# GitHubOfAndrew/TeAMOFlow

Hardware: AMD Instinct MI355X
Metric: train_interactions_per_sec (higher is better)
Workload: dtype f32

## Files before the change

### teamoflow_amd/csrc/tmf_wmrb.hip

```cpp
#include <math.h>
#include <stdlib.h>

#include <type_traits>

#include "tmf_common.h"

namespace tmf {

constexpr int kThreads = 256;
constexpr int kWaves = kThreads / 64;
constexpr int kPosChunk = 512;
constexpr int kUnrollW = 4;
constexpr int kG4Unroll = 4;

__host__ __device__ inline int round4(int x) { return (x + 3) & ~3; }

__host__ __device__ inline int sp_padded(int S) {
    const int nf4 = (S + 3) / 4;
    const int per = ((nf4 + 2 * kWaves - 1) / (2 * kWaves) + 1) & ~1;
    return 4 * 2 * kWaves * per;
}

__device__ __forceinline__ void count_ge0_x4(int& c0, int& c1, float x0, float x1, float x2, float x3) {
    unsigned long long m0, m1, m2, m3;
// ... 973 lines not shown
                       D, delta, (const T*)U_old, U_out, epi, adam, b, e, sy, lag)
        TMF_DISPATCH(T, geom, CALL);
#undef CALL
    }
    return check_launch("tmf_wmrb_gradu4");
}


namespace tmf {
constexpr int kS5Users = 256;
constexpr int kS5Waves = 15;
constexpr int kS5Pad = INT32_MIN;
constexpr int kS5MaxWindows = 4096;
constexpr int kS5Stride = 16;

struct S5Pace {
    const int32_t* wst;
    int* cnt;
    int nw, lag;
};

template <int NV, typename T>
__global__ __launch_bounds__(64 * (kS5Waves + 1)) void k_wmrb_scores5(const int32_t* __restrict__ ids, const int32_t* __restrict__ outs,
                                                                     const int64_t* __restrict__ wg_ptr, int64_t wg0, int64_t n_users,
                                                                     const T* __restrict__ U, const T* __restrict__ V,
                                                                     float* __restrict__ sp, float* __restrict__ p, S5Pace pace) {
    constexpr int G = 32, NGB = 2 * kS5Waves;
    constexpr uint32_t RB = RowBytes<G, NV, T>::value;
    extern __shared__ __attribute__((aligned(16))) char smem_raw[];
    __shared__ int s_win[kS5Waves];
    __shared__ int s_gate;
    int* wst = reinterpret_cast<int*>(smem_raw + (size_t)kS5Users * RB);
    const int tid = threadIdx.x, lane = tid & 63, wave = tid >> 6, g = lane & (G - 1), gid = tid / G;
    const int64_t wg = wg0 + blockIdx.x;
    const int64_t ubeg = wg * kS5Users;
    const int nu = (int)((n_users - ubeg < kS5Users) ? n_users - ubeg : kS5Users);
    const bool paced = pace.cnt != nullptr;
    {
        const tmf_f4* src = reinterpret_cast<const tmf_f4*>(reinterpret_cast<const char*>(U) + ubeg * (int64_t)RB);
        tmf_f4* dst = reinterpret_cast<tmf_f4*>(smem_raw);
        for (int i = tid; i < nu * (int)(RB / 16); i += 64 * (kS5Waves + 1)) dst[i] = __builtin_nontemporal_load(src + i);
        if (paced)
            for (int i = tid; i <= pace.nw; i += 64 * (kS5Waves + 1)) wst[i] = pace.wst[wg * (pace.nw + 1) + i];
        if (tid < kS5Waves) s_win[tid] = 0;
        if (tid == 0) s_gate = paced ? pace.lag : INT32_MAX;
    }
    __syncthreads();
    if (wave == kS5Waves) {
        if (!paced) return;
        const int x = blockIdx.x & 7, peers = ((int)gridDim.x - x + 7) / 8;
        int* cnt = pace.cnt + (size_t)x * pace.nw * kS5Stride;
        int published = 0, gate = pace.lag, idle = 0;
        bool open = false;
        for (;;) {
            int mn = (lane < kS5Waves) ? __hip_atomic_load(&s_win[lane], __ATOMIC_RELAXED, __HIP_MEMORY_SCOPE_WORKGROUP) : INT32_MAX;
#pragma unroll
            for (int o = 8; o >= 1; o >>= 1) mn = min(mn, __shfl_xor(mn, o, 64));
            mn = __builtin_amdgcn_readfirstlane(mn);
            const bool done = mn == INT32_MAX;
            const int target = done ? pace.nw : mn;
            if (lane == 0)
                for (int w = published; w < target; ++w) __hip_atomic_fetch_add(cnt + (size_t)w * kS5Stride, 1, __ATOMIC_RELAXED, __HIP_MEMORY_SCOPE_AGENT);
            if (target > published) published = target;
            if (done) return;
            if (!open && gate < pace.nw - 1) {
                int c = (lane == 0) ? __hip_atomic_load(cnt + (size_t)(gate - pace.lag) * kS5Stride, __ATOMIC_RELAXED, __HIP_MEMORY_SCOPE_AGENT) : 0;
                c = __builtin_amdgcn_readfirstlane(c);
                if (c >= peers) {
                    ++gate;
                    idle = 0;
                    if (lane == 0) __hip_atomic_store(&s_gate, gate, __ATOMIC_RELAXED, __HIP_MEMORY_SCOPE_WORKGROUP);
                    continue;
                }
                if (++idle > 4000) {
                    open = true;
                    if (lane == 0) __hip_atomic_store(&s_gate, INT32_MAX, __ATOMIC_RELAXED, __HIP_MEMORY_SCOPE_WORKGROUP);
                }
            }
            __builtin_amdgcn_s_sleep(4);
        }
    }
    const int64_t beg = wg_ptr[wg], end = wg_ptr[wg + 1];
    const int steps = (int)((end - beg) >> 3);
    const uint32_t loff = 16u * (uint32_t)g;
    const int my_entry = Reduce8x32::entry_of_lane(lane);
    const bool owner = Reduce8x32::owner(lane);
    const int4* id4 = reinterpret_cast<const int4*>(ids + beg);
    const int32_t* out8 = outs + beg + my_entry;
    const int mine = steps > gid ? (steps - gid + NGB - 1) / NGB : 0;
    const int rounds = __builtin_amdgcn_readfirstlane(mine);
    if (rounds > 0) {
        const int last = mine > 0 ? gid + NGB * (mine - 1) : 0;
        struct Ids {
            int4 a, b;
            int o;
        };
        auto fetch = [&](int i) {
            const int st = gid + NGB * i;
            const int sc = st <= last ? st : last;
            Ids r{id4[2 * sc], id4[2 * sc + 1], out8[8 * sc]};
            if (i >= mine) r.o = kS5Pad;
            return r;
        };
        int cur_w = 0, next_b = paced ? wst[1] : INT32_MAX;
        auto pace_to = [&](int i) {
            if (!paced || i >= rounds || cur_w >= pace.nw - 1) return;
            const int st_w = __builtin_amdgcn_readfirstlane(gid + NGB * i);
            if (st_w < next_b) return;
            do {
                ++cur_w;
                next_b = wst[cur_w + 1];
            } while (st_w >= next_b && cur_w < pace.nw - 1);
            if (lane == 0) __hip_atomic_store(&s_win[wave], cur_w, __ATOMIC_RELAXED, __HIP_MEMORY_SCOPE_WORKGROUP);
            for (int spin = 0; spin < 20000; ++spin) {
                if (__hip_atomic_load(&s_gate, __ATOMIC_RELAXED, __HIP_MEMORY_SCOPE_WORKGROUP) >= cur_w) break;
                __builtin_amdgcn_s_sleep(2);
            }
        };
        auto gather = [&](Raw<NV, T> (&y)[8], const Ids& d) {
            const int idv[8] = {d.a.x, d.a.y, d.a.z, d.a.w, d.b.x, d.b.y, d.b.z, d.b.w};
#pragma unroll
            for (int t = 0; t < 8; ++t) load_raw32<G, NV>(y[t], V, (uint32_t)idv[t] & 0xffffffu, loff);
        };
        auto finish = [&](const Raw<NV, T> (&y)[8], const Ids& d) {
            const int idv[8] = {d.a.x, d.a.y, d.a.z, d.a.w, d.b.x, d.b.y, d.b.z, d.b.w};
            float pr[8];
#pragma unroll
            for (int t = 0; t < 8; ++t) {
                Raw<NV, T> x;
                const char* xr = smem_raw + ((uint32_t)idv[t] >> 24) * RB + loff;
                if constexpr (std::is_same<T, float>::value) {
#pragma unroll
                    for (int v = 0; v < NV; ++v) x.v[v] = *reinterpret_cast<const float4*>(xr + 16 * G * v);
                } else {
#pragma unroll
                    for (int pv = 0; pv < NV / 2; ++pv) x.v[pv] = *reinterpret_cast<const bf16x8*>(xr + 16 * G * pv);
                }
                pr[t] = dot_raw<NV>(x, y[t]);
            }
            const float sc = Reduce8x32::run(pr, lane);
            if (owner && d.o != kS5Pad) __builtin_nontemporal_store(sc, d.o >= 0 ? sp + d.o : p + ~d.o);
        };
        Raw<NV, T> yA[8], yB[8];
        Ids A = fetch(0);
        Ids B = fetch(1);
        pace_to(0);
        gather(yA, A);
        for (int i = 0; i < rounds; i += 2) {
            Ids C = fetch(i + 2);
            __builtin_amdgcn_sched_barrier(0);
            pace_to(i + 1);
            gather(yB, B);
            __builtin_amdgcn_sched_barrier(0);
            finish(yA, A);
            __builtin_amdgcn_sched_barrier(0);
            if (i + 1 >= rounds) break;
            Ids Dn = fetch(i + 3);
            __builtin_amdgcn_sched_barrier(0);
            pace_to(i + 2);
            gather(yA, C);
            __builtin_amdgcn_sched_barrier(0);
            finish(yB, B);
            __builtin_amdgcn_sched_barrier(0);
            A = C;
            B = Dn;
        }
    }
    if (lane == 0) __hip_atomic_store(&s_win[wave], INT32_MAX, __ATOMIC_RELAXED, __HIP_MEMORY_SCOPE_WORKGROUP);
}

}

namespace tmf {
constexpr int kS6Users = 64;
constexpr int kS6Waves = 8;

template <int NV, typename T>
__global__ __launch_bounds__(64 * kS6Waves) void k_wmrb_scores6(const int32_t* __restrict__ ids, const int32_t* __restrict__ outs,
                                                                const int64_t* __restrict__ chunk_ptr, int64_t chunk0, int64_t n_groups,
                                                                int64_t n_users, const T* __restrict__ U, const T* __restrict__ V,
                                                                float* __restrict__ sp, float* __restrict__ p) {
    constexpr int G = 32, NGB = 2 * kS6Waves;
    constexpr uint32_t RB = RowBytes<G, NV, T>::value;
    __shared__ __attribute__((aligned(16))) char smem_raw[kS6Users * RB];
    const int tid = threadIdx.x, lane = tid & 63, g = lane & (G - 1), gid = tid / G;
    const int64_t chunk = chunk0 + blockIdx.x;
    const int64_t beg = chunk_ptr[chunk], end = chunk_ptr[chunk + 1];
    if (beg == end) return;
    const int64_t ubeg = (chunk % n_groups) * kS6Users;
    const int nu = (int)((n_users - ubeg < kS6Users) ? n_users - ubeg : kS6Users);
    {
        const tmf_f4* src = reinterpret_cast<const tmf_f4*>(reinterpret_cast<const char*>(U) + ubeg * (int64_t)RB);
        tmf_f4* dst = reinterpret_cast<tmf_f4*>(smem_raw);
        for (int i = tid; i < nu * (int)(RB / 16); i += 64 * kS6Waves) dst[i] = __builtin_nontemporal_load(src + i);
    }
    __syncthreads();
    const int steps = (int)((end - beg) >> 3);
    const uint32_t loff = 16u * (uint32_t)g;
    const int my_entry = Reduce8x32::entry_of_lane(lane);
    const bool owner = Reduce8x32::owner(lane);
    const int4* id4 = reinterpret_cast<const int4*>(ids + beg);
    const int32_t* out8 = outs + beg + my_entry;
    const int mine = steps > gid ? (steps - gid + NGB - 1) / NGB : 0;
    const int rounds = __builtin_amdgcn_readfirstlane(mine);
    if (rounds == 0) return;
    const int last = mine > 0 ? gid + NGB * (mine - 1) : 0;
    struct Ids {
        int4 a, b;
        int o;
    };
    auto fetch = [&](int i) {
        const int st = gid + NGB * i;
        const int sc = st <= last ? st : last;
        Ids r{id4[2 * sc], id4[2 * sc + 1], out8[8 * sc]};
        if (i >= mine) r.o = kS5Pad;
        return r;
    };
    auto gather = [&](Raw<NV, T> (&y)[8], const Ids& d) {
        const int idv[8] = {d.a.x, d.a.y, d.a.z, d.a.w, d.b.x, d.b.y, d.b.z, d.b.w};
#pragma unroll
        for (int t = 0; t < 8; ++t) load_raw32<G, NV>(y[t], V, (uint32_t)idv[t] & 0xffffffu, loff);
    };
    auto finish = [&](const Raw<NV, T> (&y)[8], const Ids& d) {
        const int idv[8] = {d.a.x, d.a.y, d.a.z, d.a.w, d.b.x, d.b.y, d.b.z, d.b.w};
        float pr[8];
#pragma unroll
        for (int t = 0; t < 8; ++t) {
            Raw<NV, T> x;
            const char* xr = smem_raw + ((uint32_t)idv[t] >> 24) * RB + loff;
            if constexpr (std::is_same<T, float>::value) {
#pragma unroll
                for (int v = 0; v < NV; ++v) x.v[v] = *reinterpret_cast<const float4*>(xr + 16 * G * v);
            } else {
#pragma unroll
                for (int pv = 0; pv < NV / 2; ++pv) x.v[pv] = *reinterpret_cast<const bf16x8*>(xr + 16 * G * pv);
            }
            pr[t] = dot_raw<NV>(x, y[t]);
        }
        const float sc = Reduce8x32::run(pr, lane);
        if (owner && d.o != kS5Pad) __builtin_nontemporal_store(sc, d.o >= 0 ? sp + d.o : p + ~d.o);
    };
    Raw<NV, T> yA[8];
    Ids A = fetch(0);
    for (int i = 0; i < rounds; ++i) {
        Ids B = fetch(i + 1);
        __builtin_amdgcn_sched_barrier(0);
        gather(yA, A);
        __builtin_amdgcn_sched_barrier(0);
        finish(yA, A);
        A = B;
    }
}

}

static bool s6_supported(int n_components, int bf16, int64_t n_items) {
    const tmf::RowGeom geom = bf16 ? tmf::row_geom_bf16(n_components) : tmf::row_geom(n_components);
    const int64_t row_bytes = (int64_t)geom.ld * (bf16 ? 2 : 4);
    return geom.G == 32 && n_items > 0 && n_items < (1 << 24) && n_items * row_bytes < ((int64_t)1 << 32);
}

template <typename T>
static int wmrb_scores6_impl(const int32_t* ids, const int32_t* outs, const int64_t* chunk_ptr, int64_t n_groups, int32_t n_slices,
                             int64_t n_users, int64_t n_items, const void* U, const void* V, float* sp, float* p, int n_components,
                             void* stream) {
    if (n_users == 0 || n_slices == 0) return TMF_OK;
    const RowGeom geom = row_geom_of<T>(n_components);
    TMF_REQUIRE(ids && outs && chunk_ptr && U && V && sp && p, "wmrb_scores6: null pointer");
    TMF_REQUIRE(n_groups == (n_users + kS6Users - 1) / kS6Users && n_slices > 0, "wmrb_scores6: %lld groups for %lld users (%d per group), %d slices",
                (long long)n_groups, (long long)n_users, kS6Users, n_slices);
    if (!s6_supported(n_components, std::is_same<T, __bf16>::value, n_items)) {
        set_error("wmrb_scores6: needs rows of 32 lanes (fp32 65..128 / bf16 129..256 components) and fewer than 2^24 items in a table "
                  "below 4 GB (got %d components, %lld items)", n_components, (long long)n_items);
        return TMF_E_UNSUPPORTED;
    }
    const int64_t per_slice = n_groups * 64 * kS6Waves;
    const int max_slices = (int)((((int64_t)1 << 32) - 1) / per_slice);
    TMF_REQUIRE(max_slices >= 1, "wmrb_scores6: %lld user groups exceed one launch", (long long)n_groups);
    for (int s0 = 0; s0 < n_slices; s0 += max_slices) {
        const int nsl = (n_slices - s0 < max_slices) ? n_slices - s0 : max_slices;
        const unsigned blocks = (unsigned)(n_groups * nsl);
#define CALL(G_, NV_)                                                                                                       \
    {                                                                                                                       \
        if constexpr (G_ == 32) {                                                                                           \
            hipLaunchKernelGGL((k_wmrb_scores6<NV_, T>), dim3(blocks), dim3(64 * kS6Waves), 0, (hipStream_t)stream, ids, outs, \
                               chunk_ptr, (int64_t)s0 * n_groups, n_groups, n_users, (const T*)U, (const T*)V, sp, p);      \
        }                                                                                                                   \
    }
        TMF_DISPATCH(T, geom, CALL);
#undef CALL
    }
    return check_launch("tmf_wmrb_scores6");
}

namespace tmf {
constexpr int kS7Users = 256;
constexpr int kS7Slots = 6144;
constexpr int kS7K = 4;
constexpr int kS7Waves = 16;
constexpr int kS7Flight = 2;
constexpr uint32_t kS7RowBytes = 512;
constexpr size_t kS7Lds = (size_t)kS7Users * kS7RowBytes + (size_t)(kS7Slots + 64) * sizeof(float);

struct S7Streams {
    const int4* steps;
    const int32_t* place;
    const int64_t* sub_step;
    const int64_t* sub_place;
    const int32_t* chunk_sub;
    const int32_t* sub_wave;
    const int32_t* sub_fill;
};

__global__ __launch_bounds__(64 * kS7Waves) void k_wmrb_scores7(S7Streams a, int64_t chunk0, int64_t n_groups, int64_t n_users,
                                                                const float* __restrict__ U, const float* __restrict__ V,
                                                                float* __restrict__ sp, float* __restrict__ p) {
    constexpr int NG = 8 * kS7Waves, NT = 64 * kS7Waves, FL = kS7Flight;
    extern __shared__ __attribute__((aligned(16))) char smem_raw[];
    float* sbuf = reinterpret_cast<float*>(smem_raw + (size_t)kS7Users * kS7RowBytes);
    const int tid = threadIdx.x, lane = tid & 63, g = lane & 7, gid = tid >> 3;
    const int64_t chunk = chunk0 + blockIdx.x;
    const int sub_b = a.chunk_sub[chunk], sub_e = a.chunk_sub[chunk + 1];
    if (sub_b == sub_e) return;
    const int64_t ubeg = (chunk % n_groups) * kS7Users;
    const int nu = (int)((n_users - ubeg < kS7Users) ? n_users - ubeg : kS7Users);
    {
        const tmf_f4* src = reinterpret_cast<const tmf_f4*>(reinterpret_cast<const char*>(U) + ubeg * (int64_t)kS7RowBytes);
        tmf_f4* dst = reinterpret_cast<tmf_f4*>(smem_raw);
        for (int i = tid; i < nu * (int)(kS7RowBytes / 16); i += NT) dst[i] = __builtin_nontemporal_load(src + i);
    }
    __syncthreads();
    const uint32_t par = (lane >> 4) & 1;
    const uint32_t offA = 16u * g + 128u * par, offB = 16u * g + 128u * (par ^ 1u);
    const uint32_t slot_sel = 0x0c0c0000u | ((2u * (g & 3) + 1u) << 8) | (2u * (g & 3));
    struct Row {
        float4 v[4];
    };
    auto dot = [](const Row& x, const Row& y) {
        float q[4];
#pragma unroll
        for (int v = 0; v < 4; ++v) {
            tmf_f2 a = tmf_f2{x.v[v].x, x.v[v].y} * tmf_f2{y.v[v].x, y.v[v].y};
            a = __builtin_elementwise_fma(tmf_f2{x.v[v].z, x.v[v].w}, tmf_f2{y.v[v].z, y.v[v].w}, a);
            q[v] = a.x + a.y;
        }
        return (q[0] + q[2]) + (q[1] + q[3]);
    };
    auto run = [&](auto fill_tag, const int4* rec0, int first, int stride, int end, int rounds) {
        constexpr int FILL = decltype(fill_tag)::value;
        auto fetch = [&](int i) {
            const int st = first + stride * i;
            return rec0[st < end ? st : end - 1];
        };
        auto gather = [&](Row& y, const int4& r) {
            const char* base = reinterpret_cast<const char*>(V);
            const uint32_t oa = row_byte_off<kS7RowBytes>((uint32_t)r.x, offA), ob = row_byte_off<kS7RowBytes>((uint32_t)r.x, offB);
            y.v[0] = *reinterpret_cast<const float4*>(base + oa);
            y.v[1] = *reinterpret_cast<const float4*>(base + ob);
            y.v[2] = *reinterpret_cast<const float4*>(base + oa + 256);
            y.v[3] = *reinterpret_cast<const float4*>(base + ob + 256);
        };
        auto finish = [&](const Row& y, const int4& r, int i) {
            float s[FILL];
#pragma unroll
            for (int k = 0; k < FILL; ++k) {
                const uint32_t lu = ((uint32_t)r.y >> (8 * k)) & 0xffu;
                const char* xa = smem_raw + (lu * kS7RowBytes + offA);
                const char* xb = smem_raw + (lu * kS7RowBytes + offB);
                Row x;
                x.v[0] = *reinterpret_cast<const float4*>(xa);
                x.v[1] = *reinterpret_cast<const float4*>(xb);
                x.v[2] = *reinterpret_cast<const float4*>(xa + 256);
                x.v[3] = *reinterpret_cast<const float4*>(xb + 256);
                float t = dot(x, y);
                t += TMF_DPP_MOV(t, 0xB1);
                t += TMF_DPP_MOV(t, 0x4E);
                t += TMF_DPP_MOV(t, 0x141);
                s[k] = t;
            }
            float mine_s = s[0];
            if constexpr (FILL == 2) mine_s = (g & 1) ? s[1] : s[0];
            if constexpr (FILL == 3) mine_s = (g & 2) ? s[2] : ((g & 1) ? s[1] : s[0]);
            if constexpr (FILL == 4) mine_s = (g & 2) ? ((g & 1) ? s[3] : s[2]) : ((g & 1) ? s[1] : s[0]);
            uint32_t slot = __builtin_amdgcn_perm((uint32_t)r.w, (uint32_t)r.z, slot_sel);
            slot = (slot < (uint32_t)kS7Slots && first + stride * i < end) ? slot : (uint32_t)kS7Slots;
            if (g < FILL) sbuf[slot] = mine_s;
        };
        Row y[FL];
        int4 rec[2 * FL];
#pragma unroll
        for (int j = 0; j < FL; ++j) rec[j] = fetch(j);
#pragma unroll
        for (int j = 0; j < FL; ++j) {
            gather(y[j], rec[j]);
            rec[FL + j] = fetch(FL + j);
        }
        int i = 0;
        for (; i + 2 * FL <= rounds; i += 2 * FL) {
#pragma unroll
            for (int j = 0; j < 2 * FL; ++j) {
                __builtin_amdgcn_sched_barrier(0);
                finish(y[j % FL], rec[j], i + j);
                __builtin_amdgcn_sched_barrier(0);
                gather(y[j % FL], rec[(j + FL) % (2 * FL)]);
                rec[j] = fetch(i + j + 2 * FL);
            }
        }
        const int rem = rounds - i;
#pragma unroll
        for (int j = 0; j < 2 * FL - 1; ++j) {
            if (j < rem) {
                __builtin_amdgcn_sched_barrier(0);
                finish(y[j % FL], rec[j], i + j);
                __builtin_amdgcn_sched_barrier(0);
                if (j + FL < rem) gather(y[j % FL], rec[j + FL]);
            }
        }
    };
    const int wave = __builtin_amdgcn_readfirstlane(tid >> 6);
    const bool by_fill = a.sub_wave != nullptr;
    for (int sub = sub_b; sub < sub_e; ++sub) {
        const int64_t st0 = a.sub_step[sub];
        const int nsteps = (int)(a.sub_step[sub + 1] - st0);
        const int64_t pl0 = a.sub_place[sub];
        const int nslots = (int)(a.sub_place[sub + 1] - pl0);
        const int4* rec0 = a.steps + st0;
        const int32_t* pl = a.place + pl0;
        int32_t where[kS7Slots / NT];
#pragma unroll
        for (int q = 0; q < kS7Slots / NT; ++q) where[q] = (tid + NT * q < nslots) ? __builtin_nontemporal_load(pl + tid + NT * q) : 0;
        int lo = 8 * wave, hi = nsteps, stride = NG, wb = 0, we = 0, cls = 0;
        if (by_fill) {
            const int32_t* sw = a.sub_wave + (int64_t)sub * (kS7Waves + 1) + wave;
            wb = __builtin_amdgcn_readfirstlane(sw[0]);
            we = __builtin_amdgcn_readfirstlane(sw[1]);
            cls = __builtin_amdgcn_readfirstlane(a.sub_fill[(int64_t)sub * kS7K]);
            lo = wb, hi = we < cls ? we : cls, stride = 8;
        }
        if (lo < hi) run(std::integral_constant<int, 4>{}, rec0, lo + (by_fill ? (gid & 7) : gid - 8 * wave), stride, hi, (hi - lo + stride - 1) / stride);
        if (by_fill) {
            const int32_t* sf = a.sub_fill + (int64_t)sub * kS7K;
            int end = cls + __builtin_amdgcn_readfirstlane(sf[1]);
            lo = wb > cls ? wb : cls, hi = we < end ? we : end, cls = end;
            if (lo < hi) run(std::integral_constant<int, 3>{}, rec0, lo + (gid & 7), 8, hi, (hi - lo + 7) / 8);
            end = cls + __builtin_amdgcn_readfirstlane(sf[2]);
            lo = wb > cls ? wb : cls, hi = we < end ? we : end, cls = end;
            if (lo < hi) run(std::integral_constant<int, 2>{}, rec0, lo + (gid & 7), 8, hi, (hi - lo + 7) / 8);
            lo = wb > cls ? wb : cls, hi = we;
            if (lo < hi) run(std::integral_constant<int, 1>{}, rec0, lo + (gid & 7), 8, hi, (hi - lo + 7) / 8);
        }
        __syncthreads();
#pragma unroll
        for (int q = 0; q < kS7Slots / NT; ++q)
            if (tid + NT * q < nslots)
                __builtin_nontemporal_store(sbuf[tid + NT * q], where[q] >= 0 ? sp + where[q] : p + ~where[q]);
        __syncthreads();
    }
}

}

static bool s7_supported(int n_components, int bf16, int64_t n_items) {
    return !bf16 && n_components >= 65 && n_components <= 128 && s6_supported(n_components, 0, n_items);
}

static int wmrb_scores7_impl(const void* steps, const int32_t* place, const int64_t* sub_step, const int64_t* sub_place,
                             const int32_t* chunk_sub, const int32_t* sub_wave, const int32_t* sub_fill, int64_t n_groups, int32_t n_slices, int64_t n_users, int64_t n_items,
                             const void* U, const void* V, float* sp, float* p, int n_components, void* stream) {
    if (n_users == 0 || n_slices == 0) return TMF_OK;
    TMF_REQUIRE(steps && place && sub_step && sub_place && chunk_sub && U && V && sp && p, "wmrb_scores7: null pointer");
    TMF_REQUIRE(!sub_wave == !sub_fill, "wmrb_scores7: sub_wave and sub_fill come together");
    TMF_REQUIRE(n_groups == (n_users + kS7Users - 1) / kS7Users && n_slices > 0, "wmrb_scores7: %lld groups for %lld users (%d per group), %d slices",
                (long long)n_groups, (long long)n_users, kS7Users, n_slices);
    if (!s7_supported(n_components, 0, n_items)) {
        set_error("wmrb_scores7: needs fp32 rows of 65..128 components and fewer than 2^24 items in a table below 4 GB "
                  "(got %d components, %lld items)", n_components, (long long)n_items);
        return TMF_E_UNSUPPORTED;
    }
    static LdsGrant grant;
    if (int rc = grant_dynamic_lds(reinterpret_cast<const void*>(&k_wmrb_scores7), kS7Lds, grant)) return rc;
    const S7Streams a{static_cast<const int4*>(steps), place, sub_step, sub_place, chunk_sub, sub_wave, sub_fill};
    const int64_t per_slice = n_groups * 64 * kS7Waves;
    const int max_slices = (int)((((int64_t)1 << 32) - 1) / per_slice);
    TMF_REQUIRE(max_slices >= 1, "wmrb_scores7: %lld user groups exceed one launch", (long long)n_groups);
    for (int s0 = 0; s0 < n_slices; s0 += max_slices) {
        const int nsl = (n_slices - s0 < max_slices) ? n_slices - s0 : max_slices;
        hipLaunchKernelGGL(k_wmrb_scores7, dim3((unsigned)(n_groups * nsl)), dim3(64 * kS7Waves), kS7Lds, (hipStream_t)stream, a,
                           (int64_t)s0 * n_groups, n_groups, n_users, (const float*)U, (const float*)V, sp, p);
    }
    return check_launch("tmf_wmrb_scores7");
}

static int s5_launches(int64_t n_wg, int wgs_per_launch) { return (int)((n_wg + wgs_per_launch - 1) / wgs_per_launch); }
static int s5_wgs_per_launch(int wgs_per_launch) {
    if (wgs_per_launch > 0) return wgs_per_launch;
    int dev = 0, cus = 256;
    if (hipGetDevice(&dev) == hipSuccess) (void)hipDeviceGetAttribute(&cus, hipDeviceAttributeMultiprocessorCount, dev);
    return cus > 0 ? cus : 256;
}

template <typename T>
static int wmrb_scores5_impl(const int32_t* ids, const int32_t* outs, const int64_t* wg_ptr, int64_t n_wg, int64_t n_users,
                             int64_t n_items, const void* U, const void* V, float* sp, float* p, int n_components,
                             int wgs_per_launch, const int32_t* wstart, int32_t n_windows, int lag, void* workspace,
                             size_t workspace_bytes, void* stream) {
    if (n_wg == 0 || n_users == 0) return TMF_OK;
    const RowGeom geom = row_geom_of<T>(n_components);
    TMF_REQUIRE(ids && outs && wg_ptr && U && V && sp && p, "wmrb_scores5: null pointer");
    TMF_REQUIRE(n_wg == (n_users + kS5Users - 1) / kS5Users, "wmrb_scores5: %lld workgroups for %lld users (%d per workgroup)",
                (long long)n_wg, (long long)n_users, kS5Users);
    const size_t row_bytes = (size_t)geom.ld * sizeof(T);
    if (geom.G != 32 || row_bytes * kS5Users > 128 * 1024 || n_items <= 0 || n_items >= (1 << 24) ||
        (int64_t)n_items * (int64_t)row_bytes >= ((int64_t)1 << 32)) {
        set_error("wmrb_scores5: needs rows of 32 lanes (fp32 65..128 / bf16 129..256 components) and fewer than 2^24 items "
                  "in a table below 4 GB (got %d components, %lld items)", n_components, (long long)n_items);
        return TMF_E_UNSUPPORTED;
    }
    wgs_per_launch = s5_wgs_per_launch(wgs_per_launch);
    const int launches = s5_launches(n_wg, wgs_per_launch);
    const bool paced = wstart != nullptr && workspace != nullptr && n_windows > 1;
    const size_t per_launch = (size_t)8 * (paced ? n_windows : 0) * kS5Stride * sizeof(int);
    if (paced) {
        TMF_REQUIRE(n_windows <= kS5MaxWindows && lag >= 0, "wmrb_scores5: %d windows (at most %d), lag %d", n_windows, kS5MaxWindows, lag);
        TMF_REQUIRE(workspace_bytes >= per_launch * launches, "wmrb_scores5: workspace of %zu bytes needed, got %zu", per_launch * launches,
                    workspace_bytes);
        if (hipMemsetAsync(workspace, 0, per_launch * launches, (hipStream_t)stream) != hipSuccess) {
            set_error("wmrb_scores5: hipMemsetAsync failed");
            return TMF_E_LAUNCH;
        }
    }
    const size_t lds = row_bytes * kS5Users + (paced ? (size_t)(n_windows + 1) * sizeof(int) : 0);
#define CALL(G_, NV_)                                                                                                       \
    {                                                                                                                       \
        if constexpr (G_ == 32) {                                                                                           \
            static LdsGrant grant;                                                                                          \
            if (int rc = grant_dynamic_lds(reinterpret_cast<const void*>(&k_wmrb_scores5<NV_, T>), lds, grant)) return rc;  \
            for (int l = 0; l < launches; ++l) {                                                                            \
                const int64_t w0 = (int64_t)l * wgs_per_launch;                                                             \
                const unsigned blocks = (unsigned)((n_wg - w0 < wgs_per_launch) ? n_wg - w0 : wgs_per_launch);              \
                const S5Pace pace{wstart, paced ? reinterpret_cast<int*>(static_cast<char*>(workspace) + per_launch * l) : nullptr, \
                                  n_windows, lag};                                                                          \
                hipLaunchKernelGGL((k_wmrb_scores5<NV_, T>), dim3(blocks), dim3(64 * (kS5Waves + 1)), lds, (hipStream_t)stream, \
                                   ids, outs, wg_ptr, w0, n_users, (const T*)U, (const T*)V, sp, p, pace);                  \
            }                                                                                                               \
        }                                                                                                                   \
    }
    TMF_DISPATCH(T, geom, CALL);
#undef CALL
    return check_launch("tmf_wmrb_scores5");
}

template <typename T>
static int wmrb_finish_impl(const float* part, int32_t n_slices, int32_t n_users, const void* U_old, void* U_out,
                            int n_components, int epi, tmf_adam adam, void* stream) {
    if (n_users == 0) return TMF_OK;
    TMF_REQUIRE(part && U_out && n_slices > 0 && (epi == TMF_EPI_GRAD || U_old), "wmrb_finish: bad arguments");
    TMF_REQUIRE(epi == TMF_EPI_ADAM || epi == TMF_EPI_GRAD, "wmrb_finish: bad epilogue %d", epi);
    const RowGeom geom = row_geom_of<T>(n_components);
#define CALL(G_, NV_)                                                                                                  \
    {                                                                                                                  \
        constexpr int per_block = (64 / G_) * kWaves;                                                                  \
        hipLaunchKernelGGL((k_wmrb_finish<G_, NV_, T>), dim3((unsigned)(((int64_t)n_users + per_block - 1) / per_block)), \
                           dim3(kThreads), 0, (hipStream_t)stream, part, (int)n_slices, (int64_t)n_users,                \
                           (const T*)U_old, U_out, epi, adam);                                                         \
    }
    TMF_DISPATCH(T, geom, CALL);
#undef CALL
    return check_launch("tmf_wmrb_finish");
}

#define TMF_SLICED_ENTRY_POINTS(SFX, T_)                                                                                  \
    extern "C" int tmf_wmrb_scores3_##SFX(const tmf_slice_lists* lists, const void* U, const void* V, float* sp, float* p, \
                                          int n_components, void* stream) {                                               \
        return wmrb_scores3_impl<T_>(lists, U, V, sp, p, n_components, stream);                                           \
    }                                                                                                                     \
    extern "C" int tmf_wmrb_scores5_##SFX(const int32_t* ids, const int32_t* outs, const int64_t* wg_ptr, int64_t n_wg,    \
                                          int64_t n_users, int64_t n_items, const void* U, const void* V, float* sp,      \
                                          float* p, int n_components, int wgs_per_launch, const int32_t* wstart,          \
                                          int32_t n_windows, int lag, void* workspace, size_t workspace_bytes,            \
                                          void* stream) {                                                                 \
        return wmrb_scores5_impl<T_>(ids, outs, wg_ptr, n_wg, n_users, n_items, U, V, sp, p, n_components, wgs_per_launch, \
                                     wstart, n_windows, lag, workspace, workspace_bytes, stream);                         \
    }                                                                                                                     \
    extern "C" int tmf_wmrb_scores6_##SFX(const int32_t* ids, const int32_t* outs, const int64_t* chunk_ptr, int64_t n_groups, \
                                          int32_t n_slices, int64_t n_users, int64_t n_items, const void* U, const void* V, \
                                          float* sp, float* p, int n_components, void* stream) {                          \
        return wmrb_scores6_impl<T_>(ids, outs, chunk_ptr, n_groups, n_slices, n_users, n_items, U, V, sp, p, n_components, stream); \
    }                                                                                                                     \
    extern "C" int tmf_wmrb_gradu3_##SFX(const tmf_slice_lists* lists, const float* D, const float* delta,                \
                                         const void* V, float* part, int per_slice_launches, int n_components,            \
                                         void* stream) {                                                                  \
        return wmrb_gradu3_impl<T_>(lists, D, delta, V, part, per_slice_launches, n_components, stream);                  \
    }                                                                                                                     \
    extern "C" int tmf_wmrb_gradu4_##SFX(const tmf_slice_lists* lists, const float* D, const float* delta, const void* V,  \
                                         const void* U_old, void* U_out, int n_components, int epi, tmf_adam adam,       \
                                         int32_t users_per_launch, void* workspace, size_t workspace_bytes, void* stream) { \
        return wmrb_gradu4_impl<T_>(lists, D, delta, V, U_old, U_out, n_components, epi, adam, users_per_launch, workspace, \
                                    workspace_bytes, stream);                                                            \
    }                                                                                                                     \
    extern "C" int tmf_wmrb_finish_##SFX(const float* part, int32_t n_slices, int32_t n_users, const void* U_old,         \
                                         void* U_out, int n_components, int epi, tmf_adam adam, void* stream) {           \
        return wmrb_finish_impl<T_>(part, n_slices, n_users, U_old, U_out, n_components, epi, adam, stream);               \
    }

TMF_SLICED_ENTRY_POINTS(f32, float)
TMF_SLICED_ENTRY_POINTS(bf16, __bf16)

extern "C" int tmf_wmrb_scores6_users_per_group(void) { return tmf::kS6Users; }
extern "C" int tmf_wmrb_scores6_supported(int n_components, int bf16, int64_t n_items) { return s6_supported(n_components, bf16, n_items); }
extern "C" int tmf_wmrb_scores7_f32(const void* steps, const int32_t* place, const int64_t* sub_step, const int64_t* sub_place,
                                    const int32_t* chunk_sub, int64_t n_groups, int32_t n_slices, int64_t n_users, int64_t n_items,
                                    const void* U, const void* V, float* sp, float* p, int n_components, void* stream) {
    return wmrb_scores7_impl(steps, place, sub_step, sub_place, chunk_sub, nullptr, nullptr, n_groups, n_slices, n_users, n_items, U, V, sp, p,
                             n_components, stream);
}
extern "C" int tmf_wmrb_scores7_fill_f32(const void* steps, const int32_t* place, const int64_t* sub_step, const int64_t* sub_place,
                                         const int32_t* chunk_sub, const int32_t* sub_wave, const int32_t* sub_fill, int64_t n_groups,
                                         int32_t n_slices, int64_t n_users, int64_t n_items, const void* U, const void* V, float* sp,
                                         float* p, int n_components, void* stream) {
    TMF_REQUIRE(sub_wave && sub_fill, "wmrb_scores7_fill: null pointer");
    return wmrb_scores7_impl(steps, place, sub_step, sub_place, chunk_sub, sub_wave, sub_fill, n_groups, n_slices, n_users, n_items, U, V,
                             sp, p, n_components, stream);
}
extern "C" int tmf_wmrb_scores7_waves(void) { return tmf::kS7Waves; }
extern "C" int tmf_wmrb_scores7_users_per_group(void) { return tmf::kS7Users; }
extern "C" int tmf_wmrb_scores7_slots(void) { return tmf::kS7Slots; }
extern "C" int tmf_wmrb_scores7_supported(int n_components, int bf16, int64_t n_items) { return s7_supported(n_components, bf16, n_items); }
extern "C" int tmf_wmrb_scores5_users_per_workgroup(void) { return tmf::kS5Users; }
extern "C" size_t tmf_wmrb_scores5_workspace_bytes(int64_t n_wg, int32_t n_windows, int wgs_per_launch) {
    if (n_wg <= 0 || n_windows <= 1) return 0;
    return (size_t)s5_launches(n_wg, s5_wgs_per_launch(wgs_per_launch)) * 8 * (size_t)n_windows * tmf::kS5Stride * sizeof(int);
}
extern "C" int tmf_wmrb_scores5_supported(int n_components, int bf16, int64_t n_items) {
    const tmf::RowGeom geom = bf16 ? tmf::row_geom_bf16(n_components) : tmf::row_geom(n_components);
    const int64_t row_bytes = (int64_t)geom.ld * (bf16 ? 2 : 4);
    return geom.G == 32 && row_bytes * tmf::kS5Users <= 128 * 1024 && n_items > 0 && n_items < (1 << 24) &&
           n_items * row_bytes < ((int64_t)1 << 32);
}
```

Before: 1.270 billion.

## Pipeline WMRB scores7 across sub-chunks with a unified software-pipelined step stream

Replaces the per-sub-chunk run() loops, each with its own prologue and drain, with a single continuous software pipeline. Record fetches and V-row gathers for the next sub-chunk (and the next fill class) are issued while the current one finishes, and the next sub-chunk's placement indices are prefetched before the flush barrier. Sub-chunk metadata comes in through inline scalar-load asm, and the barriers are lighter waitcnt+s_barrier pairs. The aim is to remove pipeline bubbles at sub-chunk and fill-class boundaries. In exchange it adds runtime fill dispatch per step, more register state, and fragile inline asm.

Result: no change. 1.282 billion, median of 6 (+1.0%).

```diff
diff --git a/teamoflow_amd/csrc/tmf_wmrb.hip b/teamoflow_amd/csrc/tmf_wmrb.hip
--- a/teamoflow_amd/csrc/tmf_wmrb.hip
+++ b/teamoflow_amd/csrc/tmf_wmrb.hip
@@ -1299,6 +1299,30 @@
 constexpr uint32_t kS7RowBytes = 512;
 constexpr size_t kS7Lds = (size_t)kS7Users * kS7RowBytes + (size_t)(kS7Slots + 64) * sizeof(float);
 
+__device__ __forceinline__ void s7_open(const int64_t* ss, const int64_t* spl, int64_t& st0, int64_t& st1, int64_t& pl0, int64_t& pl1) {
+    asm volatile("s_load_dwordx2 %0, %4, 0x0\n\ts_load_dwordx2 %1, %4, 0x8\n\ts_load_dwordx2 %2, %5, 0x0\n\ts_load_dwordx2 %3, %5, 0x8\n\t"
+                 "s_waitcnt lgkmcnt(0)"
+                 : "=&s"(st0), "=&s"(st1), "=&s"(pl0), "=&s"(pl1) : "s"(ss), "s"(spl));
+}
+__device__ __forceinline__ void s7_open(const int64_t* ss, const int64_t* spl, const int32_t* sw, const int32_t* sf, int64_t& st0,
+                                        int64_t& pl0, int64_t& pl1, int& wb, int& we, int& n4, int& n3, int& n2) {
+    asm volatile("s_load_dwordx2 %0, %8, 0x0\n\ts_load_dwordx2 %1, %9, 0x0\n\ts_load_dwordx2 %2, %9, 0x8\n\t"
+                 "s_load_dword %3, %10, 0x0\n\ts_load_dword %4, %10, 0x4\n\t"
+                 "s_load_dword %5, %11, 0x0\n\ts_load_dword %6, %11, 0x4\n\ts_load_dword %7, %11, 0x8\n\ts_waitcnt lgkmcnt(0)"
+                 : "=&s"(st0), "=&s"(pl0), "=&s"(pl1), "=&s"(wb), "=&s"(we), "=&s"(n4), "=&s"(n3), "=&s"(n2)
+                 : "s"(ss), "s"(spl), "s"(sw), "s"(sf));
+}
+__device__ __forceinline__ void s7_words(const int64_t* ptr, int64_t& x, int64_t& y) {
+    asm volatile("s_load_dwordx2 %0, %2, 0x0\n\ts_load_dwordx2 %1, %2, 0x8\n\ts_waitcnt lgkmcnt(0)" : "=&s"(x), "=&s"(y) : "s"(ptr));
+}
+
+__device__ __forceinline__ void s7_barrier() {
+    asm volatile("" ::: "memory");
+    __builtin_amdgcn_s_waitcnt(0xc07f);
+    __builtin_amdgcn_s_barrier();
+    asm volatile("" ::: "memory");
+}
+
 struct S7Streams {
     const int4* steps;
     const int32_t* place;
@@ -1343,115 +1367,141 @@
         }
         return (q[0] + q[2]) + (q[1] + q[3]);
     };
-    auto run = [&](auto fill_tag, const int4* rec0, int first, int stride, int end, int rounds) {
+    const int wave = __builtin_amdgcn_readfirstlane(tid >> 6);
+    const int g8 = gid & 7;
+    const bool by_fill = a.sub_wave != nullptr;
+    const int64_t step_first = a.sub_step[sub_b];
+    int fsub = sub_b - 1, frem = 0, fbase = 0, fend = 1, fstride = 0, fc1 = 0, fc2 = 0, fc3 = 0, fnone = 7, psub = -1, pn = 0;
+    int64_t pl0 = 0;
+    const int4* frec0 = a.steps + step_first;
+    auto advance = [&]() __attribute__((always_inline)) {
+        const bool more = fsub + 1 < sub_e;
+        fsub = more ? fsub + 1 : fsub;
+        int64_t st0, st1, first, end;
+        int wb, we, stride, c1, c2, c3, rounds;
+        if (by_fill) {
+            int n4, n3, n2;
+            s7_open(a.sub_step + fsub, a.sub_place + fsub, a.sub_wave + (int64_t)fsub * (kS7Waves + 1) + wave, a.sub_fill + (int64_t)fsub * kS7K,
+                    st0, first, end, wb, we, n4, n3, n2);
+            stride = 8, c1 = n4, c2 = n4 + n3, c3 = n4 + n3 + n2;
+            rounds = we > wb ? (we - wb + 7) >> 3 : 1;
+        } else {
+            s7_open(a.sub_step + fsub, a.sub_place + fsub, st0, st1, first, end);
+            wb = 8 * wave, we = (int)(st1 - st0), stride = NG;
+            c1 = c2 = c3 = 0x7fffffff;
+            rounds = we > wb ? (we - wb + NG - 1) / NG : 1;
+        }
+        frec0 = a.steps + (more ? st0 : step_first);
+        fbase = more ? wb : 0, fend = more ? we : 1, fstride = more ? stride : 0;
+        fc1 = more ? c1 : 0, fc2 = more ? c2 : 0, fc3 = more ? c3 : 0;
+        frem = more ? rounds : 0, fnone = more ? 7 : 0;
+        psub = more ? fsub : -1, pl0 = first, pn = (int)(end - first);
+    };
+    auto fetch = [&](int4& r, int& nvalid, int& fill, int& last) __attribute__((always_inline)) {
+        if (frem == 0) advance();
+        int st = fbase + g8;
+        st = st < fend ? st : fend - 1;
+        r = frec0[st > 0 ? st : 0];
+        nvalid = fend - fbase;
+        fill = (fbase < fc1 ? 4 : (fbase < fc2 ? 3 : (fbase < fc3 ? 2 : 1))) & fnone;
+        last = frem == 1;
+        fbase += fstride;
+        frem -= frem > 0;
+    };
+    auto gather = [&](Row& y, const int4& r) {
+        const char* base = reinterpret_cast<const char*>(V);
+        const uint32_t oa = row_byte_off<kS7RowBytes>((uint32_t)r.x, offA), ob = row_byte_off<kS7RowBytes>((uint32_t)r.x, offB);
+        y.v[0] = *reinterpret_cast<const float4*>(base + oa);
+        y.v[1] = *reinterpret_cast<const float4*>(base + ob);
+        y.v[2] = *reinterpret_cast<const float4*>(base + oa + 256);
+        y.v[3] = *reinterpret_cast<const float4*>(base + ob + 256);
+    };
+    auto finish = [&](auto fill_tag, const Row& y, const int4& r, int nvalid) {
         constexpr int FILL = decltype(fill_tag)::value;
-        auto fetch = [&](int i) {
-            const int st = first + stride * i;
-            return rec0[st < end ? st : end - 1];
-        };
-        auto gather = [&](Row& y, const int4& r) {
-            const char* base = reinterpret_cast<const char*>(V);
-            const uint32_t oa = row_byte_off<kS7RowBytes>((uint32_t)r.x, offA), ob = row_byte_off<kS7RowBytes>((uint32_t)r.x, offB);
-            y.v[0] = *reinterpret_cast<const float4*>(base + oa);
-            y.v[1] = *reinterpret_cast<const float4*>(base + ob);
-            y.v[2] = *reinterpret_cast<const float4*>(base + oa + 256);
-            y.v[3] = *reinterpret_cast<const float4*>(base + ob + 256);
-        };
-        auto finish = [&](const Row& y, const int4& r, int i) {
-            float s[FILL];
-#pragma unroll
-            for (int k = 0; k < FILL; ++k) {
-                const uint32_t lu = ((uint32_t)r.y >> (8 * k)) & 0xffu;
-                const char* xa = smem_raw + (lu * kS7RowBytes + offA);
-                const char* xb = smem_raw + (lu * kS7RowBytes + offB);
-                Row x;
-                x.v[0] = *reinterpret_cast<const float4*>(xa);
-                x.v[1] = *reinterpret_cast<const float4*>(xb);
-                x.v[2] = *reinterpret_cast<const float4*>(xa + 256);
-                x.v[3] = *reinterpret_cast<const float4*>(xb + 256);
-                float t = dot(x, y);
-                t += TMF_DPP_MOV(t, 0xB1);
-                t += TMF_DPP_MOV(t, 0x4E);
-                t += TMF_DPP_MOV(t, 0x141);
-                s[k] = t;
-            }
-            float mine_s = s[0];
-            if constexpr (FILL == 2) mine_s = (g & 1) ? s[1] : s[0];
-            if constexpr (FILL == 3) mine_s = (g & 2) ? s[2] : ((g & 1) ? s[1] : s[0]);
-            if constexpr (FILL == 4) mine_s = (g & 2) ? ((g & 1) ? s[3] : s[2]) : ((g & 1) ? s[1] : s[0]);
-            uint32_t slot = __builtin_amdgcn_perm((uint32_t)r.w, (uint32_t)r.z, slot_sel);
-            slot = (slot < (uint32_t)kS7Slots && first + stride * i < end) ? slot : (uint32_t)kS7Slots;
-            if (g < FILL) sbuf[slot] = mine_s;
-        };
-        Row y[FL];
-        int4 rec[2 * FL];
-#pragma unroll
-        for (int j = 0; j < FL; ++j) rec[j] = fetch(j);
-#pragma unroll
-        for (int j = 0; j < FL; ++j) {
-            gather(y[j], rec[j]);
-            rec[FL + j] = fetch(FL + j);
-        }
-        int i = 0;
-        for (; i + 2 * FL <= rounds; i += 2 * FL) {
-#pragma unroll
-            for (int j = 0; j < 2 * FL; ++j) {
-                __builtin_amdgcn_sched_barrier(0);
-                finish(y[j % FL], rec[j], i + j);
-                __builtin_amdgcn_sched_barrier(0);
-                gather(y[j % FL], rec[(j + FL) % (2 * FL)]);
-                rec[j] = fetch(i + j + 2 * FL);
-            }
-        }
-        const int rem = rounds - i;
-#pragma unroll
-        for (int j = 0; j < 2 * FL - 1; ++j) {
-            if (j < rem) {
-                __builtin_amdgcn_sched_barrier(0);
-                finish(y[j % FL], rec[j], i + j);
-                __builtin_amdgcn_sched_barrier(0);
-                if (j + FL < rem) gather(y[j % FL], rec[j + FL]);
-            }
-        }
+        float s[FILL];
+#pragma unroll
+        for (int k = 0; k < FILL; ++k) {
+            const uint32_t lu = ((uint32_t)r.y >> (8 * k)) & 0xffu;
+            const char* xa = smem_raw + (lu * kS7RowBytes + offA);
+            const char* xb = smem_raw + (lu * kS7RowBytes + offB);
+            Row x;
+            x.v[0] = *reinterpret_cast<const float4*>(xa);
+            x.v[1] = *reinterpret_cast<const float4*>(xb);
+            x.v[2] = *reinterpret_cast<const float4*>(xa + 256);
+            x.v[3] = *reinterpret_cast<const float4*>(xb + 256);
+            float t = dot(x, y);
+            t += TMF_DPP_MOV(t, 0xB1);
+            t += TMF_DPP_MOV(t, 0x4E);
+            t += TMF_DPP_MOV(t, 0x141);
+            s[k] = t;
+        }
+        float mine_s = s[0];
+        if constexpr (FILL == 2) mine_s = (g & 1) ? s[1] : s[0];
+        if constexpr (FILL == 3) mine_s = (g & 2) ? s[2] : ((g & 1) ? s[1] : s[0]);
+        if constexpr (FILL == 4) mine_s = (g & 2) ? ((g & 1) ? s[3] : s[2]) : ((g & 1) ? s[1] : s[0]);
+        uint32_t slot = __builtin_amdgcn_perm((uint32_t)r.w, (uint32_t)r.z, slot_sel);
+        slot = (slot < (uint32_t)kS7Slots && g8 < nvalid) ? slot : (uint32_t)kS7Slots;
+        if (g < FILL) sbuf[slot] = mine_s;
     };
-    const int wave = __builtin_amdgcn_readfirstlane(tid >> 6);
-    const bool by_fill = a.sub_wave != nullptr;
-    for (int sub = sub_b; sub < sub_e; ++sub) {
-        const int64_t st0 = a.sub_step[sub];
-        const int nsteps = (int)(a.sub_step[sub + 1] - st0);
-        const int64_t pl0 = a.sub_place[sub];
-        const int nslots = (int)(a.sub_place[sub + 1] - pl0);
-        const int4* rec0 = a.steps + st0;
-        const int32_t* pl = a.place + pl0;
-        int32_t where[kS7Slots / NT];
-#pragma unroll
-        for (int q = 0; q < kS7Slots / NT; ++q) where[q] = (tid + NT * q < nslots) ? __builtin_nontemporal_load(pl + tid + NT * q) : 0;
-        int lo = 8 * wave, hi = nsteps, stride = NG, wb = 0, we = 0, cls = 0;
-        if (by_fill) {
-            const int32_t* sw = a.sub_wave + (int64_t)sub * (kS7Waves + 1) + wave;
-            wb = __builtin_amdgcn_readfirstlane(sw[0]);
-            we = __builtin_amdgcn_readfirstlane(sw[1]);
-            cls = __builtin_amdgcn_readfirstlane(a.sub_fill[(int64_t)sub * kS7K]);
-            lo = wb, hi = we < cls ? we : cls, stride = 8;
-        }
-        if (lo < hi) run(std::integral_constant<int, 4>{}, rec0, lo + (by_fill ? (gid & 7) : gid - 8 * wave), stride, hi, (hi - lo + stride - 1) / stride);
-        if (by_fill) {
-            const int32_t* sf = a.sub_fill + (int64_t)sub * kS7K;
-            int end = cls + __builtin_amdgcn_readfirstlane(sf[1]);
-            lo = wb > cls ? wb : cls, hi = we < end ? we : end, cls = end;
-            if (lo < hi) run(std::integral_constant<int, 3>{}, rec0, lo + (gid & 7), 8, hi, (hi - lo + 7) / 8);
-            end = cls + __builtin_amdgcn_readfirstlane(sf[2]);
-            lo = wb > cls ? wb : cls, hi = we < end ? we : end, cls = end;
-            if (lo < hi) run(std::integral_constant<int, 2>{}, rec0, lo + (gid & 7), 8, hi, (hi - lo + 7) / 8);
-            lo = wb > cls ? wb : cls, hi = we;
-            if (lo < hi) run(std::integral_constant<int, 1>{}, rec0, lo + (gid & 7), 8, hi, (hi - lo + 7) / 8);
-        }
-        __syncthreads();
+    int32_t where[kS7Slots / NT], ahead[kS7Slots / NT];
+    int nslots = 0, nslots_ahead = 0;
+    auto places = [&](int64_t first, int n) __attribute__((always_inline)) {
+        nslots_ahead = n;
+        const int32_t* pl = a.place + first;
+#pragma unroll
+        for (int q = 0; q < kS7Slots / NT; ++q)
+            ahead[q] = __builtin_nontemporal_load(pl + (tid + NT * q < n ? tid + NT * q : (n > 0 ? n - 1 : 0)));
+    };
+    auto flush = [&](int sub) __attribute__((always_inline)) {
+#pragma unroll
+        for (int q = 0; q < kS7Slots / NT; ++q) asm volatile("v_mov_b32 %0, %1" : "=v"(where[q]) : "v"(ahead[q]));
+        nslots = nslots_ahead;
+        if (sub + 1 < sub_e) {
+            if (psub == sub + 1) {
+                places(pl0, pn);
+            } else {
+                int64_t first, end;
+                s7_words(a.sub_place + sub + 1, first, end);
+                places(first, (int)(end - first));
+            }
+        }
+        s7_barrier();
 #pragma unroll
         for (int q = 0; q < kS7Slots / NT; ++q)
             if (tid + NT * q < nslots)
                 __builtin_nontemporal_store(sbuf[tid + NT * q], where[q] >= 0 ? sp + where[q] : p + ~where[q]);
-        __syncthreads();
+        s7_barrier();
+    };
+    Row y[FL];
+    int4 rec[2 * FL];
+    int nvalid[2 * FL], fill[2 * FL], last[2 * FL];
+    advance();
+    places(pl0, pn);
+#pragma unroll
+    for (int j = 0; j < FL; ++j) fetch(rec[j], nvalid[j], fill[j], last[j]);
+#pragma unroll
+    for (int j = 0; j < FL; ++j) {
+        gather(y[j], rec[j]);
+        fetch(rec[FL + j], nvalid[FL + j], fill[FL + j], last[FL + j]);
+    }
+    int csub = sub_b, due = 0;
+    while (csub < sub_e) {
+#pragma unroll
+        for (int j = 0; j < 2 * FL; ++j) {
+            if (due) {
+                flush(csub);
+                ++csub;
+            }
+            due = last[j];
+            __builtin_amdgcn_sched_barrier(0);
+            if (fill[j] == 4) finish(std::integral_constant<int, 4>{}, y[j % FL], rec[j], nvalid[j]);
+            else if (fill[j] == 3) finish(std::integral_constant<int, 3>{}, y[j % FL], rec[j], nvalid[j]);
+            else if (fill[j] == 2) finish(std::integral_constant<int, 2>{}, y[j % FL], rec[j], nvalid[j]);
+            else if (fill[j] == 1) finish(std::integral_constant<int, 1>{}, y[j % FL], rec[j], nvalid[j]);
+            __builtin_amdgcn_sched_barrier(0);
+            gather(y[j % FL], rec[(j + FL) % (2 * FL)]);
+            fetch(rec[j], nvalid[j], fill[j], last[j]);
+        }
     }
 }
 
```
